# fanzhongyi/ExploreMultiModal

Measured on AMD Instinct MI355X. Metric: image-text pairs/sec fwd+bwd, VLMo-Base, 1/2/4/8 MI355X; % bf16 MFMA roofline, higher is better.
Workload: dtype bf16

## Files before the change

### exploremultimodal_amd/csrc/block.hip

```cpp
#include "common.h"
#include "vlmo_hip.h"
#include <algorithm>
#include <map>
#include <vector>

namespace {
constexpr int GELU_DERIV = 4;


struct Events {
    std::vector<hipEvent_t> pool;
    hipEvent_t get(size_t i) {
        while (pool.size() <= i) {
            hipEvent_t e = nullptr;
            (void)hipEventCreateWithFlags(&e, hipEventDisableTiming);
            pool.push_back(e);
        }
        return pool[i];
    }
};
Events& events() {
    static thread_local std::map<int, Events> per_device;
    int dev = 0;
    (void)hipGetDevice(&dev);
// ... 289 lines not shown
    arm();
    TRY(vlmo_ln_bwd(b->dy1, 0, nullptr, b->x, b->n1w, b->mean1, b->rstd1, b->dx1, b->dx0, b->dn1w, b->dn1b, M, d,
                    ws_slot(2 + b->n_experts), slot, st));
    collect();
    return 0;
}

}

extern "C" int vlmo_stack_fwd(const VlmoStackDesc* s, hipStream_t st) {
    VLMO_CHECK_ARG(s && s->blocks && s->n_blocks >= 1, "vlmo_stack_fwd: empty stack");
    for (int i = 0; i < s->n_blocks; ++i)
        if (int rc = block_fwd(&s->blocks[i], st)) return rc;
    return 0;
}

extern "C" int vlmo_stack_bwd(const VlmoStackDesc* s, hipStream_t st) {
    VLMO_CHECK_ARG(s && s->blocks && s->n_blocks >= 1, "vlmo_stack_bwd: empty stack");
    const int nb = s->n_blocks;
    const int batch = s->wgrad_batch >= 1 ? s->wgrad_batch : 1;
    const int nsets = s->n_tmp_sets >= 1 ? s->n_tmp_sets : 1;
    hipStream_t side = s->side_stream ? s->side_stream : st;
    const bool two = side != st;
    VLMO_CHECK_ARG(!two || nsets > batch || nb <= nsets,
                   "vlmo_stack_bwd: %d temporary sets cannot cover deferred batches of %d blocks", nsets, batch);
    Events& ev = events();
    Deferred D;
    D.store = s->wgrad_store != 0;
    std::vector<int> batch_of(nb, -1);
    int n_batches = 0, waited_upto = -1;
    auto flush = [&]() -> int {
        if (D.blocks.empty()) return 0;
        if (two) {
            hipEvent_t f = ev.get(2 * n_batches);
            (void)hipEventRecord(f, st);
            (void)hipStreamWaitEvent(side, f, 0);
        }
        std::stable_sort(D.tn.begin(), D.tn.end(), [](const VlmoTnProblem& a, const VlmoTnProblem& b) { return a.M > b.M; });
        TRY(vlmo_gemm_tn_multi(VLMO_BF16, D.tn.data(), (int)D.tn.size(), side));
        TRY(vlmo_colwork_multi(VLMO_BF16, D.col.data(), (int)D.col.size(), side));
        if (two) (void)hipEventRecord(ev.get(2 * n_batches + 1), side);
        if (s->grad_ready)
            for (int i : D.blocks)
                if (s->grad_ready[i]) (void)hipEventRecord((hipEvent_t)s->grad_ready[i], side);
        ++n_batches;
        D.tn.clear();
        D.col.clear();
// ... 49 lines not shown
```

### exploremultimodal_amd/csrc/gemm_tn.hip

```cpp
#include "gemm_common.h"
#include <algorithm>
#include <vector>

namespace {

struct GemmTN {
    const void* A;
    const void* B;
    float* C;
    int M, N1, N2, lda, ldb, ldc;
    int kt_per_split, tiles;
    float alpha;
    float* slab;
    int mode;
};
enum { TN_ATOMIC = 0, TN_ACCUM = 1, TN_STORE = 2 };

__device__ __attribute__((aligned(256))) char tn_zero_page[256];

__device__ __forceinline__ int tn_swz(int row) { return ((row & 3) << 2) | ((row >> 2) & 3); }

template <typename T, int BM, int BN, int WM, int WN, bool PP = false>
__device__ __forceinline__ void gemm_tn_body(const GemmTN& p, const int lid) {
    typedef typename Elem<T>::v8 v8;
// ... 217 lines not shown
        for (int j = 0; j < TN; ++j) {
            const int gn = n2_0 + wn * (BN / WN) + j * 32 + l31;
#pragma unroll
            for (int r = 0; r < 16; ++r) {
                const int gm = n1_0 + wm * (BM / WM) + i * 32 + (r & 3) + 8 * (r >> 2) + 4 * h;
                if (gm < p.N1 && gn < p.N2) {
                    float* c = p.C + (size_t)gm * p.ldc + gn;
                    if (p.slab)
                        p.slab[((size_t)split * p.N1 + gm) * p.N2 + gn] = acc[i][j][r];
                    else if (p.mode == TN_STORE)
                        *c = p.alpha * acc[i][j][r];
                    else
                        atomicAdd(c, p.alpha * acc[i][j][r]);
                }
            }
        }
}

template <typename T, int BM, int BN, int WM, int WN, bool PP = false>
__global__ __launch_bounds__(WM * WN * 64, 2) void gemm_tn_kernel(const GemmTN p) {
    gemm_tn_body<T, BM, BN, WM, WN, PP>(p, xcd_remap(blockIdx.x, gridDim.x));
}

constexpr int MAX_TN_PROBS = 16;
constexpr int MAX_TN_ORDER = 1024;
constexpr uint16_t TN_NOP = 0xFFFF;
struct GemmTNMulti {
    int n;
    GemmTN p[MAX_TN_PROBS];
    uint16_t order[MAX_TN_ORDER];
};
template <typename T>
__global__ __launch_bounds__(512, 2) void gemm_tn_multi_kernel(const GemmTNMulti mp) {
    const uint32_t code = mp.order[blockIdx.x];
    if (code == TN_NOP) return;
    int gi = (int)(code >> 12);
    const int lid_in = __builtin_amdgcn_readfirstlane((int)(code & 0xFFFu));
    gi = __builtin_amdgcn_readfirstlane(gi);
    const GemmTN& q = mp.p[gi];
    GemmTN p;
    p.A = uniform_ptr(q.A), p.B = uniform_ptr(q.B), p.C = (float*)uniform_ptr(q.C);
    p.M = __builtin_amdgcn_readfirstlane(q.M), p.N1 = __builtin_amdgcn_readfirstlane(q.N1);
    p.N2 = __builtin_amdgcn_readfirstlane(q.N2), p.lda = __builtin_amdgcn_readfirstlane(q.lda);
    p.ldb = __builtin_amdgcn_readfirstlane(q.ldb), p.ldc = __builtin_amdgcn_readfirstlane(q.ldc);
    p.kt_per_split = __builtin_amdgcn_readfirstlane(q.kt_per_split), p.tiles = __builtin_amdgcn_readfirstlane(q.tiles);
    p.alpha = __builtin_bit_cast(float, __builtin_amdgcn_readfirstlane(__builtin_bit_cast(int, q.alpha)));
    p.slab = nullptr;
    p.mode = __builtin_amdgcn_readfirstlane(q.mode);
    gemm_tn_body<T, 256, 256, 2, 4, true>(p, lid_in);
}

__global__ __launch_bounds__(256) void tn_reduce_kernel(const float* __restrict__ slab, int splits, int N1, int N2,
                                                        float* __restrict__ C, int ldc, float alpha) {
    const int n4 = N2 >> 2;
    const long total = (long)N1 * n4;
    for (long i = (long)blockIdx.x * 256 + threadIdx.x; i < total; i += (long)gridDim.x * 256) {
        const int r = (int)(i / n4), c = (int)(i % n4) * 4;
        f32x4 a = {0.f, 0.f, 0.f, 0.f};
        for (int s2 = 0; s2 < splits; ++s2) a += *(const f32x4*)(slab + ((size_t)s2 * N1 + r) * N2 + c);
        f32x4* o = (f32x4*)(C + (size_t)r * ldc + c);
        *o = *o + alpha * a;
    }
// ... 58 lines not shown
            (void)hipFuncSetAttribute((const void*)gemm_tn_kernel<bf16, 256, 256, 2, 4, true>, hipFuncAttributeMaxDynamicSharedMemorySize, LDS);
            (void)hipFuncSetAttribute((const void*)gemm_tn_kernel<f16, 256, 256, 2, 4, true>, hipFuncAttributeMaxDynamicSharedMemorySize, LDS);
        }
        if (dtype == VLMO_F16)
            hipLaunchKernelGGL((gemm_tn_kernel<f16, 256, 256, 2, 4, true>), grid, dim3(512), LDS, stream, p);
        else
            hipLaunchKernelGGL((gemm_tn_kernel<bf16, 256, 256, 2, 4, true>), grid, dim3(512), LDS, stream, p);
    } else {
        if (dtype == VLMO_F16)
            hipLaunchKernelGGL((gemm_tn_kernel<f16, 128, 128, 2, 2>), grid, dim3(256), 65536, stream, p);
        else
            hipLaunchKernelGGL((gemm_tn_kernel<bf16, 128, 128, 2, 2>), grid, dim3(256), 65536, stream, p);
    }
    VLMO_CHECK_LAUNCH("vlmo_gemm_tn");
    if (use_slab) {
        const long total = (long)N1 * (N2 / 4);
        const int rg = (int)((total + 255) / 256 < 2048 ? (total + 255) / 256 : 2048);
        hipLaunchKernelGGL(tn_reduce_kernel, dim3(rg), dim3(256), 0, stream, ws, pl.splits, N1, N2, C, ldc, alpha);
        VLMO_CHECK_LAUNCH("vlmo_gemm_tn(reduce)");
    }
    return 0;
}

extern "C" int vlmo_gemm_tn_multi(int dtype, const VlmoTnProblem* probs, int n, hipStream_t stream) {
    VLMO_CHECK_ARG(probs && n >= 1, "vlmo_gemm_tn_multi: no problems");
    VLMO_CHECK_ARG(dtype == VLMO_BF16 || dtype == VLMO_F16, "vlmo_gemm_tn_multi: dtype must be bf16 or f16");
    static DeviceOnce attr;
    if (attr.first()) {
        constexpr int LDS = 2 * 4 * 64 * 256;
        (void)hipFuncSetAttribute((const void*)gemm_tn_multi_kernel<bf16>, hipFuncAttributeMaxDynamicSharedMemorySize, LDS);
        (void)hipFuncSetAttribute((const void*)gemm_tn_multi_kernel<f16>, hipFuncAttributeMaxDynamicSharedMemorySize, LDS);
    }
    for (int q0 = 0, nq = 0; q0 < n; q0 += nq) {
        nq = 0;
        for (long tl = 0; q0 + nq < n && nq < MAX_TN_PROBS; ++nq) {
            const VlmoTnProblem& r = probs[q0 + nq];
            const long t = (long)((r.N1 + 255) / 256) * ((r.N2 + 255) / 256);
            if (nq > 0 && tl + t > MAX_TN_ORDER - 64) break;
            tl += t;
        }
        long tiles_all = 0;
        int min_nk = 1 << 30;
        double flops = 0;
        for (int q = 0; q < nq; ++q) {
            const VlmoTnProblem& r = probs[q0 + q];
            VLMO_CHECK_ARG(r.A && r.B && r.C, "vlmo_gemm_tn_multi: null operand in problem %d", q0 + q);
            VLMO_CHECK_ARG(r.M > 0 && r.N1 >= 8 && r.N2 >= 8 && r.N1 % 8 == 0 && r.N2 % 8 == 0 && r.lda % 8 == 0 &&
                               r.ldb % 8 == 0 && r.lda >= r.N1 && r.ldb >= r.N2 && r.ldc >= r.N2,
                           "vlmo_gemm_tn_multi: bad shape in problem %d (M=%d N1=%d N2=%d)", q0 + q, r.M, r.N1, r.N2);
            tiles_all += (long)((r.N1 + 255) / 256) * ((r.N2 + 255) / 256);
            const int nk = (r.M + 63) / 64;
            if (nk < min_nk) min_nk = nk;
            flops += 2.0 * r.M * r.N1 * r.N2;
        }
        int splits = 1;
        if (tiles_all < 192) {
            splits = (int)(256 / tiles_all);
            if (splits > min_nk / 8) splits = min_nk / 8;
            if (splits < 1) splits = 1;
        }
        GemmTNMulti mp{};
        mp.n = nq;
        struct Job {
            uint16_t code;
            int cost;
        };
        std::vector<Job> jobs;
        for (int q = 0; q < nq; ++q) {
            const VlmoTnProblem& r = probs[q0 + q];
            const int tiles = ((r.N1 + 255) / 256) * ((r.N2 + 255) / 256);
            const int nk = (r.M + 63) / 64;
            int sp = splits > nk ? nk : splits;
            const int per = (nk + sp - 1) / sp;
            sp = (nk + per - 1) / per;
            int mode = r.accumulate ? TN_ACCUM : TN_STORE;
            if (sp > 1) {
                mode = TN_ATOMIC;
                if (!r.accumulate) {
                    hipError_t rc = hipMemset2DAsync(r.C, (size_t)r.ldc * 4, 0, (size_t)r.N2 * 4, r.N1, stream);
                    if (rc != hipSuccess) {
                        vlmo_set_error("vlmo_gemm_tn_multi: memset failed: %s", hipGetErrorString(rc));
                        return (int)rc;
                    }
                }
            }
            VLMO_CHECK_ARG(tiles * sp <= 4096, "vlmo_gemm_tn_multi: problem %d has too many tiles", q0 + q);
            mp.p[q] = GemmTN{r.A, r.B, r.C, r.M, r.N1, r.N2, r.lda, r.ldb, r.ldc, per, tiles, r.alpha, nullptr, mode};
            for (int l = 0; l < tiles * sp; ++l) jobs.push_back(Job{(uint16_t)((q << 12) | l), per});
        }
        std::stable_sort(jobs.begin(), jobs.end(), [](const Job& a, const Job& b) { return a.cost > b.cost; });
        std::vector<uint16_t> bins[8];
        for (size_t i = 0; i < jobs.size();) {
            size_t j = i;
            while (j < jobs.size() && jobs[j].cost == jobs[i].cost) ++j;
            const size_t cnt = j - i;
            for (int x = 0; x < 8; ++x)
                for (size_t k = i + cnt * x / 8; k < i + cnt * (x + 1) / 8; ++k) bins[x].push_back(jobs[k].code);
            i = j;
        }
        size_t deepest = 0;
        for (int x = 0; x < 8; ++x) deepest = bins[x].size() > deepest ? bins[x].size() : deepest;
        VLMO_CHECK_ARG(deepest * 8 <= (size_t)MAX_TN_ORDER, "vlmo_gemm_tn_multi: %zu workgroups exceed one launch (pass fewer problems per call)",
                       jobs.size());
        const int t = (int)deepest * 8;
        for (int b = 0; b < t; ++b) {
            const std::vector<uint16_t>& bin = bins[b & 7];
            mp.order[b] = (size_t)(b >> 3) < bin.size() ? bin[b >> 3] : TN_NOP;
        }
        ProfScope prof(73, flops, stream);
        constexpr int LDS = 2 * 4 * 64 * 256;
        if (dtype == VLMO_F16)
            hipLaunchKernelGGL((gemm_tn_multi_kernel<f16>), dim3(t), dim3(512), LDS, stream, mp);
        else
            hipLaunchKernelGGL((gemm_tn_multi_kernel<bf16>), dim3(t), dim3(512), LDS, stream, mp);
        VLMO_CHECK_LAUNCH("vlmo_gemm_tn_multi");
    }
    return 0;
}
```

### exploremultimodal_amd/engine.py

```python
import ctypes
import os as _os
import sys
from collections import namedtuple

import torch

from . import hip

LN_EPS = 1e-12
GRAD_SINK = None
_ov = _os.environ.get('VLMO_OVERLAP_WGRAD')
OVERLAP_WGRAD = None if _ov is None else _ov != '0'
ONE_STREAM_ROWS = 12288


def _use_side_stream(sink, rows):
    if OVERLAP_WGRAD is not None:
        return OVERLAP_WGRAD
    return sink is not None or rows < ONE_STREAM_ROWS


DEFAULT_TILE = -1


# ... 304 lines not shown
    return [(w1, 0), (b1, hid * d), (w2, hid * d + hid), (b2, 2 * hid * d + hid)]


def _fill_grads(D, flats, d, hid, nexp):
    (dg1, dg2, dn1w, dn1b, dn2w, dn2b, dqkv_w, dproj_w, dproj_b, dqkv_b) = _carve(
        flats[0], [(d,)] * 6 + [(3 * d, d), (d, d), (d,), (3 * d,)])
    D.dg1, D.dg2, D.dn1w, D.dn1b, D.dn2w, D.dn2b = (t.data_ptr() for t in (dg1, dg2, dn1w, dn1b, dn2w, dn2b))
    D.dqkv_w, D.dproj_w, D.dproj_b, D.dqkv_b = (t.data_ptr() for t in (dqkv_w, dproj_w, dproj_b, dqkv_b))
    dexp = []
    for i in range(nexp):
        dw1, db1, dw2, db2 = _carve(flats[1 + i], [(hid, d), (hid,), (d, hid), (d,)])
        D.dw1[i], D.db1[i], D.dw2[i], D.db2[i] = dw1.data_ptr(), db1.data_ptr(), dw2.data_ptr(), db2.data_ptr()
        dexp += [dw1, db1, dw2, db2]
    return [dg1, dg2, dn1w, dn1b, dqkv_w, dqkv_b[:d], dqkv_b[2 * d:], dproj_w, dproj_b, dn2w, dn2b] + dexp


def _released(ctx_field):
    if ctx_field is None:
        raise RuntimeError('Trying to backward through an engine pass a second time: its saved activations were released '
                           'by the first backward (retain_graph=True is not supported by engine.StackFn)')


WGRAD_BATCH = int(_os.environ.get('VLMO_WGRAD_BATCH', '2'))


def wgrad_batch_for(d, hid, cus=256, max_batch=4):
    if WGRAD_BATCH > 0:
        return WGRAD_BATCH
    c = lambda n: -(-n // 256)
    tiles = c(d) * c(3 * d) + c(d) * c(d) + 2 * c(d) * c(hid)
    best, best_cost = 1, None
    for b in range(1, max_batch + 1):
        cost = -(-b * tiles // cus) / b
        if best_cost is None or cost < best_cost - 1e-9:
            best, best_cost = b, cost
    return best


TMP_SETS = 4
USE_STACK = True

_PERSIST = {}


def _persist(dev, tag, numel, dtype):
    key = (dev, torch.cuda.current_stream(dev).cuda_stream, tag)
    t = _PERSIST.get(key)
    if t is None or t.numel() < numel or t.dtype != dtype:
        t = _PERSIST[key] = torch.empty(numel, dtype=dtype, device=dev)
    return t


_EVENTS = {}


def _ready_events(dev, n):
    evs = _EVENTS.setdefault(dev, [])
    while len(evs) < n:
        evs.append(hip.event_create())
# ... 102 lines not shown
    if base is None or g.dtype != torch.float32 or base.dim() != 1 or not base.is_contiguous():
        return None
    off = (g.data_ptr() - base.data_ptr()) // 4
    if off < 0 or off + n > base.numel():
        return None
    return base[off:off + n]


def _same_views(layout, flat):
    for p_, off in layout:
        if not p_.requires_grad:
            continue
        pg = p_.grad
        if pg is None or pg.data_ptr() != flat.data_ptr() + 4 * off or not pg.is_contiguous() or pg.dtype != torch.float32:
            return False
        if getattr(p_, '_post_accumulate_grad_hooks', None) or getattr(p_, '_backward_hooks', None):
            return False
    return True


_Scratch = namedtuple('_Scratch', 'nsets batch tb ws ws_n dxs')


def _backward_scratch(dev, nb, M, d, hid, B):
    want = wgrad_batch_for(d, hid)
    nsets = max(1, min(max(TMP_SETS, want + 1), nb))
    batch = max(1, min(want, nsets - 1)) if nb > nsets else max(1, want)
    md = M * d
    tb = _persist(dev, 'tb', nsets * 11 * md, torch.bfloat16)
    slot = hip.lib().vlmo_reduce_ws_bytes(2 * d)
    ws_n = 6 * slot // 4 + (M // 16 + 4) * hid + 4 * B * d
    ws = _persist(dev, 'ws', nsets * ws_n, torch.float32)
    dxs = _persist(dev, 'dx', 3 * md, torch.float32)
    return _Scratch(nsets, batch, tb, ws, ws_n, dxs)


def _sink_buckets(sink, groups, d, hid, dev):
    akey = id(groups[0].params[0])
    aroom = group_numel(groups[0], d, hid) + ARENA_EXPERTS * group_numel(groups[1], d, hid)
    return [sink.acquire(g.params, group_numel(g, d, hid), dev, akey, aroom, layout=group_layout(g, d, hid), lazy_zero=True)
            for g in groups]


FRESH, FROM_TASK, FROM_GRAD = 0, 1, 2


def _local_bucket(g, d, hid, wanted, reg, permitted, into_grad, fresh):
    key = _group_key(g.params)
    if wanted:
        if reg is not None and key in reg:
            return reg[key], FROM_TASK
        if into_grad:
            have = _grad_flat(g.params, group_numel(g, d, hid))
            if have is not None and _same_views(group_layout(g, d, hid), have):
# ... 117 lines not shown
            ctx.metas, ctx.descs, ctx.keep, ctx.spans, ctx.groups = metas, descs, keep, spans, groups
            ctx.save_for_backward(x, *params)
            ctx.sink = GRAD_SINK
            if ctx.sink is None:
                ctx.grad_groups = [(_group_key(g.params), g.params) for blk in groups for g in blk]
            else:
                ctx.sink_groups = [[g.params for g in blk] for blk in groups]
                for blk in ctx.sink_groups:
                    for gp in blk:
                        ctx.sink.expect(gp)
        return out

    @staticmethod
    def backward(ctx, dxo):
        metas, descs, spans, groups = ctx.metas, ctx.descs, ctx.spans, ctx.groups
        _released(descs)
        x, *params = ctx.saved_tensors
        nb = len(metas)
        m0 = metas[0]
        d, hid = m0.d, m0.hidden
        M, dev = x.shape[0], x.device
        dxo = dxo.contiguous()
        sink = ctx.sink
        sc = _backward_scratch(dev, nb, M, d, hid, m0.plan.B)
        dx_in = torch.empty((M, d), dtype=torch.float32, device=dev)
        if sink is None:
            storage = _fresh_storage(sum(group_numel(g, d, hid) for blk in groups for g in blk), dev)
            reg = _task_flats(ctx) if INPLACE_ACCUM else None
            permitted, into_grad, off = _TASK_FLATS['groups'], INPLACE_ACCUM and _INTO_GRAD[0], 0
        grads_all = [None] * len(params)
        store_ok, acquired = True, []
        for k in range(nb):
            i = nb - 1 - k
            D, blk, (o, n_) = descs[i], groups[i], spans[i]
            if sink is not None:
                got = _sink_buckets(sink, blk, d, hid, dev)
            else:
                got, off = _local_buckets(blk, ctx.needs_input_grad[2 + o:2 + o + n_], d, hid, reg, permitted, into_grad,
                                          storage, off)
            store_ok = store_ok and all(fr for _, fr in got)
            acquired += [(f_, fr, g.lo > 0) for g, (f_, fr) in zip(blk, got)]
            grads = _fill_grads(D, [f_ for f_, _ in got], d, hid, len(blk) - 1)
            for g, (_, fr) in zip(blk, got):
                if fr or sink is not None:
                    grads_all[o + g.lo:o + g.hi] = grads[g.lo:g.hi]
            _split_backward_attention(D, metas[i])
            _wire_temporaries(D, k, nb, M * d, sc, dxo, dx_in)
        _zero_buckets(acquired, store_ok, d, hid)
        S = hip.StackDesc()
        S.n_blocks, S.wgrad_batch, S.n_tmp_sets, S.wgrad_store = nb, sc.batch, sc.nsets, int(store_ok)
        S.blocks = ctypes.cast(descs, ctypes.POINTER(hip.BlockDesc))
        side = _side_stream(dev) if _use_side_stream(sink, M) else None
        S.side_stream = side.cuda_stream if side is not None else None
        evs = None
        if sink is not None and side is not None:
            evs = _ready_events(dev, nb)
            arr = (ctypes.c_void_p * nb)(*evs)
            S.grad_ready = ctypes.cast(arr, ctypes.POINTER(ctypes.c_void_p))
        hip.stack_bwd(S)
        ctx.descs = ctx.keep = None
        if sink is not None:
            _hand_to_sink(sink, groups, spans, grads_all, evs)
            return (dx_in, None) + (None,) * len(params)
        return (dx_in, None, *grads_all)


class FinalNormFn(torch.autograd.Function):

    @staticmethod
    def forward(ctx, x, w, b, plan, out_shape, eps=LN_EPS):
        M, d = x.shape
        out = torch.empty(out_shape, dtype=torch.float32, device=x.device)
        mean, rstd = torch.empty(M, device=x.device), torch.empty(M, device=x.device)
        hip.ln_fwd(x, w, b, out, mean, rstd, plan.rowmap, M, d, eps)
        ctx.plan = plan
# ... 91 lines not shown
```

### exploremultimodal_amd/hip.py

```python
import ctypes
import os

import torch

_HERE = os.path.dirname(os.path.abspath(__file__))
LIB_PATH = os.environ.get('VLMO_HIP_LIB') or os.path.join(_HERE, 'lib', 'libvlmo_hip.so')

BF16, F16, F32 = 0, 1, 2
EPI_BIAS, EPI_BIAS_GELU, EPI_RESID, EPI_DGELU, EPI_F32, EPI_DUAL, EPI_ARGMAX, EPI_CE, EPI_CE_BWD = 0, 1, 2, 3, 4, 5, 6, 7, 8

_vp, _i32, _u32, _u64, _f32, _i64 = (ctypes.c_void_p, ctypes.c_int32, ctypes.c_uint32,
                                     ctypes.c_uint64, ctypes.c_float, ctypes.c_int64)


class Epilogue(ctypes.Structure):
    _fields_ = [('out', _vp), ('out2', _vp), ('bias', _vp), ('gamma', _vp),
                ('resid', _vp), ('row_scale', _vp), ('row_index', _vp), ('aux', _vp),
                ('ldo', _i32), ('ld2', _i32), ('relu', _i32),
                ('drop_thresh', _u32), ('inv_keep', _f32), ('beta', _f32),
                ('seed', _u64), ('colpart', _vp)]


_fp = _vp

# ... 59 lines not shown
    'vlmo_resid_bwd': [_vp, _vp, _vp, _vp, _vp, _vp, _vp, _vp, _i32, _i32, _u32, _f32, _u64, _vp, _i64, _vp],
    'vlmo_colsum': [_i32, _vp, _i32, _vp, _i32, _i32, _vp, _i64, _vp],
    'vlmo_cast_weight': [_i32, _vp, _i32, _i32, _vp, _vp, _vp],
    'vlmo_cast_weight_multi': [_i32, _i32, _vp, _vp, _vp, _vp, _vp, _vp],
    'vlmo_patchify': [_vp, _vp, _i32, _i32, _i32, _i32, _i32, _vp],
    'vlmo_embed_img_finish': [_vp, _vp, _vp, _vp, _vp, _vp, _vp, _i32, _i32, _i32, _u32, _f32,
                              _u64, _vp],
    'vlmo_embed_img_bwd': [_vp, _vp, _vp, _vp, _vp, _vp, _vp, _i32, _i32, _i32, _u32, _f32,
                           _u64, _vp],
    'vlmo_embed_txt_fwd': [_vp] * 10 + [_i32, _i32, _i32, _f32, _u32, _f32, _u64, _vp],
    'vlmo_embed_txt_bwd': [_vp] * 11 + [_i32, _i32, _i32, _u32, _f32, _u64, _vp],
    'vlmo_conv2d_nhwc': [_i32, _i32, _vp, _i32, _i32, _i32, _i32, _i32, _vp, _i32, _vp,
                         ctypes.POINTER(Epilogue), _vp],
    'vlmo_dvae_im2col': [_vp, _vp, _i32, _i32, _i32, _i32, _i32, _i32, _vp],
    'vlmo_maxpool2_nhwc': [_vp, _vp, _vp, _i32, _i32, _i32, _i32, _vp],
    'vlmo_argmax_reduce': [_vp, _i32, _vp, _i32, _vp],
    'vlmo_dvae_embed': [_vp, _vp, _vp, _vp, _i32, _i32, _i32, _vp],
    'vlmo_upsample2_nhwc': [_vp, _vp, _i32, _i32, _i32, _i32, _vp],
    'vlmo_dvae_out_head': [_vp, _vp, _vp, _vp, _i32, _i32, _i32, _i32, _i32, _vp],
    'vlmo_ce_reduce': [_vp, _i32, _vp, _i32, _vp, _vp, _vp, _i32, _vp],
    'vlmo_stack_fwd': [ctypes.POINTER(StackDesc), _vp],
    'vlmo_stack_bwd': [ctypes.POINTER(StackDesc), _vp],
    'vlmo_gemm_tn_multi': [_i32, ctypes.POINTER(TnProblem), _i32, _vp],
    'vlmo_colwork_multi': [_i32, ctypes.POINTER(ColJob), _i32, _vp],
    'vlmo_event_create': [ctypes.POINTER(ctypes.c_void_p)],
    'vlmo_event_destroy': [_vp],
    'vlmo_stream_wait_event': [_vp, _vp],
    'vlmo_profile_start': [_i32],
    'vlmo_gemm_nt_grouped': [_i32, _i32, _i32, _i32, _vp, _i32, _vp, _i32, _vp, _i32, _i32, _vp, _vp],
    'vlmo_mt_grad_norm': [ctypes.c_void_p, _f32, _f32, _vp, _vp, _vp],
    'vlmo_mt_adam': [ctypes.c_void_p, ctypes.c_void_p, _vp, _vp],
    'vlmo_mt_ema': [ctypes.c_void_p, _f32, _vp],
    'vlmo_mt_adam_ema': [ctypes.c_void_p, ctypes.c_void_p, _vp, _vp, _f32, _vp],
    'vlmo_side_stream_create': [_i32, ctypes.POINTER(ctypes.c_uint32), _i32, ctypes.POINTER(ctypes.c_void_p)],
    'vlmo_profile_stop': [_i32, ctypes.POINTER(ctypes.c_double), ctypes.POINTER(ctypes.c_double),
                          ctypes.POINTER(ctypes.c_int64)],
    'vlmo_gemm_nt_2src': [_i32, _i32, _i32, _vp, _i32, _i32, _f32, _vp, _i32, _vp, _i32, _i32, _i32, _i32,
                          ctypes.POINTER(Epilogue), _vp],
    'vlmo_comm_available': [],
    'vlmo_comm_unique_id': [_vp],
    'vlmo_comm_init': [ctypes.POINTER(ctypes.c_void_p), _vp, _i32, _i32],
    'vlmo_comm_destroy': [_vp],
    'vlmo_comm_count': [_vp, _vp, _vp],
    'vlmo_comm_all_reduce': [_vp, _vp, _vp, _i64, _i32, _vp],
    'vlmo_comm_reduce_scatter': [_vp, _vp, _vp, _i64, _i32, _vp],
    'vlmo_comm_all_gather': [_vp, _vp, _vp, _i64, _i32, _vp],
    'vlmo_grad_pack': [_vp, _vp, _i64, _f32, _vp],
    'vlmo_grad_unpack': [_vp, _vp, _i64, _vp],
    'vlmo_ln_gelu_fwd': [_vp, _i32, _vp, _vp, _vp, _i32, _vp, _vp, _i32, _i32, _f32, _vp],
    'vlmo_ln_gelu_bwd': [_vp, _i32, _vp, _i32, _vp, _vp, _vp, _vp, _vp, _i32, _vp, _i32, _vp, _vp, _vp, _i32, _i32, _vp,
                         _i64, _vp],
    'vlmo_vqa_bce': [_vp, _i32, _vp, _i32, _i32, _i32, _vp, _vp, _vp, _vp, _f32, _vp, _i32, _vp, _i32, _vp],
    'vlmo_isda_update': [_vp, _i32, _vp, _vp, _vp, _vp, _vp, _i32, _i32, _i32, _i32, _vp, _vp, _vp, _vp, _vp],
    'vlmo_isda_aug_fwd': [_vp, _i32, _vp, _vp, _i32, _i32, _i32, _i32, _f32, _vp, _i32, _vp, _i64, _vp],
    'vlmo_isda_aug_bwd': [_vp, _i32, _vp, _i32, _vp, _vp, _i32, _i32, _i32, _i32, _f32, _vp, _i32, _vp, _i64, _vp],
    'vlmo_sim_topk': [_vp, _i32, _vp, _i32, _i32, _i32, _i32, _i32, _f32, _i32, _vp, ctypes.c_size_t, _vp, _vp, _vp],
    'vlmo_crop_resample': [_vp, _i64, _vp, _vp, _i32, _vp, _vp, _i32, ctypes.POINTER(_f32), ctypes.POINTER(_f32), _f32, _vp,
                           _i64, _vp],
}

_lib = None
ABI_VERSION = 9

def lib():
    global _lib
    if _lib is None:
        if not os.path.exists(LIB_PATH):
            raise RuntimeError(
                f'{LIB_PATH} not found: build the HIP extension first '
                '(python -c "import __graft_entry__ as g; g.build()" or '
                'make -C exploremultimodal_amd/csrc). There is no CPU fallback.')
        L = ctypes.CDLL(LIB_PATH)
        L.vlmo_last_error.restype = ctypes.c_char_p
        L.vlmo_abi_version.restype = ctypes.c_int
        if L.vlmo_abi_version() != ABI_VERSION:
            raise RuntimeError(f'{LIB_PATH} has ABI version {L.vlmo_abi_version()}, this package needs {ABI_VERSION}: '
                               'rebuild it (make -C exploremultimodal_amd/csrc)')
        L.vlmo_reduce_ws_bytes.restype = ctypes.c_int64
        L.vlmo_reduce_ws_bytes.argtypes = [_i32]
        L.vlmo_gemm_tn_ws_bytes.restype = ctypes.c_int64
        L.vlmo_isda_ws_bytes.restype = ctypes.c_int64
        L.vlmo_isda_ws_bytes.argtypes = [_i32, _i32, _i32]
        L.vlmo_gemm_tn_ws_bytes.argtypes = [_i32, _i32, _i32]
        L.vlmo_sim_topk_ws_bytes.restype = ctypes.c_int64
        L.vlmo_sim_topk_ws_bytes.argtypes = [_i32, _i32, _i32, _i32]
# ... 246 lines not shown
def dvae_embed(ids, table, bias, out):
    vocab, n_init = table.shape
    _check(lib().vlmo_dvae_embed(_p(ids), _p(table), _p(bias), _p(out), ids.numel(), vocab, n_init, _stream()),
           'vlmo_dvae_embed')


def upsample2_nhwc(x, out, B, H, W, C):
    _check(lib().vlmo_upsample2_nhwc(_p(x), _p(out), B, H, W, C, _stream()), 'vlmo_upsample2_nhwc')


def dvae_out_head(x, w, bias, out, B, H, W):
    Cout, C = w.shape
    _check(lib().vlmo_dvae_out_head(_p(x), _p(w), _p(bias), _p(out), B, H, W, C, Cout, _stream()), 'vlmo_dvae_out_head')


def gemm_tn_multi(problems, dtype=BF16):
    n = len(problems)
    arr = (TnProblem * n)()
    for i, (A, B, C, M, N1, N2, acc) in enumerate(problems):
        arr[i] = TnProblem(_p(A), _p(B), _p(C), A.stride(0), B.stride(0), C.stride(0), M, N1, N2, 1.0, int(acc))
    _check(lib().vlmo_gemm_tn_multi(dtype, arr, n, _stream()), 'vlmo_gemm_tn_multi')


def colwork_multi(jobs, dtype=BF16):
    n = len(jobs)
    arr = (ColJob * n)()
    for i, (kind, src, rows, ncols, outs, n0) in enumerate(jobs):
        o = (ctypes.c_void_p * 4)(*[_p(t) for t in (list(outs) + [None] * 4)[:4]])
        arr[i] = ColJob(kind, src.stride(0), _p(src), rows, ncols, o, n0, 0)
    _check(lib().vlmo_colwork_multi(dtype, arr, n, _stream()), 'vlmo_colwork_multi')


def event_create():
    out = ctypes.c_void_p()
    _check(lib().vlmo_event_create(ctypes.byref(out)), 'vlmo_event_create')
    return out.value


def stream_wait_event(stream, ev):
    raw = stream.cuda_stream if hasattr(stream, 'cuda_stream') else stream
    _check(lib().vlmo_stream_wait_event(raw, ev), 'vlmo_stream_wait_event')


COMM_ID_BYTES = 128


# ... 253 lines not shown
```

### include/vlmo_hip.h

```cpp
#ifndef VLMO_HIP_H
#define VLMO_HIP_H

#include <stddef.h>
#include <stdint.h>

#ifdef __cplusplus
extern "C" {
#endif

#ifndef __HIP_PLATFORM_AMD__
typedef struct ihipStream_t* hipStream_t;
#endif

enum { VLMO_BF16 = 0, VLMO_F16 = 1, VLMO_F32 = 2 };

enum {
    VLMO_EPI_BIAS = 0,
    VLMO_EPI_BIAS_GELU = 1,
    VLMO_EPI_RESID = 2,
    VLMO_EPI_DGELU = 3,
    VLMO_EPI_F32 = 4,
    VLMO_EPI_DUAL = 5,
    VLMO_EPI_ARGMAX = 6,
    VLMO_EPI_CE = 7,
    VLMO_EPI_CE_BWD = 8
};

typedef struct VlmoEpilogue {
    void* out;
    void* out2;
    const float* bias;
    const float* gamma;
    const float* resid;
    const float* row_scale;
    const int32_t* row_index;
    const void* aux;
    int32_t ldo, ld2;
    int32_t relu;
    uint32_t drop_thresh;
    float inv_keep;
    float beta;
    uint64_t seed;
    float* colpart;
} VlmoEpilogue;

const char* vlmo_last_error(void);
#define VLMO_ABI_VERSION 9
int vlmo_abi_version(void);

int vlmo_gemm_nt(int epi, int dtype, int tile, const void* A, int lda, const void* B, int ldb,
                 int M, int N, int K, const VlmoEpilogue* e, hipStream_t stream);
int vlmo_gemm_nt_2src(int epi, int dtype, int tile, const void* A, int lda, int k1, float seg_scale, const void* A2,
                      int lda2, const void* B, int ldb, int M, int N, int K, const VlmoEpilogue* e,
                      hipStream_t stream);
int vlmo_gemm_nt_grouped(int epi, int dtype, int tile, int ngroups, const void* const* A, int lda,
                         const void* const* B, int ldb, const int32_t* M, int N, int K,
                         const VlmoEpilogue* e, hipStream_t stream);

int64_t vlmo_gemm_tn_ws_bytes(int M, int N1, int N2);
int vlmo_gemm_tn(int dtype, const void* A, int lda, const void* B, int ldb, float* C, int ldc,
                 int M, int N1, int N2, float alpha, int splits, float* ws, int64_t ws_bytes,
                 hipStream_t stream);

typedef struct VlmoTnProblem {
    const void* A;
    const void* B;
    float* C;
    int32_t lda, ldb, ldc;
    int32_t M, N1, N2;
    float alpha;
    int32_t accumulate;
} VlmoTnProblem;
int vlmo_gemm_tn_multi(int dtype, const VlmoTnProblem* probs, int n, hipStream_t stream);

int vlmo_ln_fwd(const float* x, const float* w, const float* b, void* y, int out_f32,
                float* mean, float* rstd, const int32_t* rowmap, int M, int d, float eps,
                hipStream_t stream);
int64_t vlmo_reduce_ws_bytes(int ncols);

int vlmo_ln_bwd(const void* dy, int dy_f32, const int32_t* rowmap, const float* x, const float* w,
                const float* mean, const float* rstd, const float* dres, float* dx, float* dw,
                float* db, int M, int d, float* ws, int64_t ws_bytes, hipStream_t stream);

int vlmo_ln_resid_bwd(const void* dy, const float* x, const float* w, const float* mean, const float* rstd,
                      const float* dres, float* dx, float* dw, float* db, const void* zd, const float* gamma,
                      const float* row_scale, const int32_t* row_index, void* dz, float* dgamma, float* dbias,
                      uint32_t drop_thresh, float inv_keep, uint64_t seed, int M, int d, float* ws,
                      int64_t ws_bytes, hipStream_t stream);

int vlmo_attn_fwd(const void* qkv, const int32_t* seg, int num_seq, const int32_t* keymask,
                  void* ctx, float* lse, int lse_stride, int heads, int d, int max_len,
                  float scale, uint32_t drop_thresh, float inv_keep, uint64_t seed, int mask_seq0,
                  hipStream_t stream);
int vlmo_attn_bwd(const void* qkv, const void* ctx, const void* dctx, const float* lse,
                  int lse_stride, const int32_t* seg, int num_seq, const int32_t* keymask,
                  void* dqkv, float* qv_colsum, int heads, int d, int max_len, float scale,
// ... 204 lines not shown
```

Measured before the change: 4538.

## Cache grouped wgrad GEMM tables on device and size single-stream wgrad batches by makespan

Moves the grouped TN weight-gradient GEMM's problem table and workgroup order from a kernel-argument struct into a device buffer. Plans are cached per device, stream and problem set, so repeated calls skip re-planning and re-uploading, and one launch now handles any number of problems instead of chunks of 16. When no side stream is used, the backward pass picks the deferred wgrad batch size from a predicted makespan over CU slots, bounded by a temporary-memory cap. This adds pinned/device allocations, a hash-keyed LRU cache, and more scratch memory when all blocks are batched at once.

```diff
diff --git a/exploremultimodal_amd/csrc/block.hip b/exploremultimodal_amd/csrc/block.hip
--- a/exploremultimodal_amd/csrc/block.hip
+++ b/exploremultimodal_amd/csrc/block.hip
@@ -335,7 +335,7 @@
     const int nsets = s->n_tmp_sets >= 1 ? s->n_tmp_sets : 1;
     hipStream_t side = s->side_stream ? s->side_stream : st;
     const bool two = side != st;
-    VLMO_CHECK_ARG(!two || nsets > batch || nb <= nsets,
+    VLMO_CHECK_ARG(nsets > batch || nb <= nsets,
                    "vlmo_stack_bwd: %d temporary sets cannot cover deferred batches of %d blocks", nsets, batch);
     Events& ev = events();
     Deferred D;
diff --git a/exploremultimodal_amd/csrc/gemm_tn.hip b/exploremultimodal_amd/csrc/gemm_tn.hip
--- a/exploremultimodal_amd/csrc/gemm_tn.hip
+++ b/exploremultimodal_amd/csrc/gemm_tn.hip
@@ -1,5 +1,7 @@
 #include "gemm_common.h"
 #include <algorithm>
+#include <cstring>
+#include <mutex>
 #include <vector>
 
 namespace {
@@ -263,22 +265,15 @@
     gemm_tn_body<T, BM, BN, WM, WN, PP>(p, xcd_remap(blockIdx.x, gridDim.x));
 }
 
-constexpr int MAX_TN_PROBS = 16;
-constexpr int MAX_TN_ORDER = 1024;
-constexpr uint16_t TN_NOP = 0xFFFF;
-struct GemmTNMulti {
-    int n;
-    GemmTN p[MAX_TN_PROBS];
-    uint16_t order[MAX_TN_ORDER];
-};
+constexpr int TN_LID_BITS = 16;
 template <typename T>
-__global__ __launch_bounds__(512, 2) void gemm_tn_multi_kernel(const GemmTNMulti mp) {
-    const uint32_t code = mp.order[blockIdx.x];
-    if (code == TN_NOP) return;
-    int gi = (int)(code >> 12);
-    const int lid_in = __builtin_amdgcn_readfirstlane((int)(code & 0xFFFu));
-    gi = __builtin_amdgcn_readfirstlane(gi);
-    const GemmTN& q = mp.p[gi];
+__global__ __launch_bounds__(512, 2) void gemm_tn_multi_kernel(const GemmTN* __restrict__ probs,
+                                                               const uint32_t* __restrict__ order, const int n_wg) {
+    if ((int)blockIdx.x >= n_wg) return;
+    const uint32_t code = order[blockIdx.x];
+    const int gi = __builtin_amdgcn_readfirstlane((int)(code >> TN_LID_BITS));
+    const int lid_in = __builtin_amdgcn_readfirstlane((int)(code & ((1u << TN_LID_BITS) - 1)));
+    const GemmTN& q = probs[gi];
     GemmTN p;
     p.A = uniform_ptr(q.A), p.B = uniform_ptr(q.B), p.C = (float*)uniform_ptr(q.C);
     p.M = __builtin_amdgcn_readfirstlane(q.M), p.N1 = __builtin_amdgcn_readfirstlane(q.N1);
@@ -383,98 +378,219 @@
     return 0;
 }
 
+namespace {
+
+constexpr int TN_CACHE_PER_STREAM = 32;
+
+struct TnClear {
+    float* C;
+    int ldc, N1, N2;
+};
+struct TnTable {
+    int device = -1;
+    hipStream_t stream = nullptr;
+    uint64_t hash = 0, used = 0;
+    std::vector<VlmoTnProblem> key;
+    char* dev = nullptr;
+    char* host = nullptr;
+    size_t cap = 0, order_off = 0;
+    hipEvent_t uploaded = nullptr;
+    int n_wg = 0;
+    double flops = 0;
+    std::vector<TnClear> clears;
+};
+struct TnCache {
+    std::mutex mu;
+    std::vector<TnTable*> tables;
+    uint64_t clock = 0;
+    int64_t uploads = 0, hits = 0;
+};
+TnCache& tn_cache() {
+    static TnCache* c = new TnCache;
+    return *c;
+}
+static_assert(sizeof(VlmoTnProblem) == 56, "VlmoTnProblem has padding: compare the cache key field by field");
+
+uint64_t tn_hash(const VlmoTnProblem* probs, int n) {
+    const uint64_t* w = (const uint64_t*)probs;
+    uint64_t h = 0xcbf29ce484222325ull ^ (uint64_t)n;
+    for (size_t i = 0; i < (size_t)n * (sizeof(VlmoTnProblem) / 8); ++i) h = (h ^ w[i]) * 0x100000001b3ull;
+    return h;
+}
+
+int tn_plan_multi(const VlmoTnProblem* probs, int n, std::vector<GemmTN>& recs, std::vector<uint32_t>& order,
+                  std::vector<TnClear>& clears, double* flops_out) {
+    long tiles_all = 0;
+    int min_nk = 1 << 30;
+    double flops = 0;
+    VLMO_CHECK_ARG(n < (1 << (32 - TN_LID_BITS)), "vlmo_gemm_tn_multi: %d problems exceed one call", n);
+    for (int q = 0; q < n; ++q) {
+        const VlmoTnProblem& r = probs[q];
+        VLMO_CHECK_ARG(r.A && r.B && r.C, "vlmo_gemm_tn_multi: null operand in problem %d", q);
+        VLMO_CHECK_ARG(r.M > 0 && r.N1 >= 8 && r.N2 >= 8 && r.N1 % 8 == 0 && r.N2 % 8 == 0 && r.lda % 8 == 0 &&
+                           r.ldb % 8 == 0 && r.lda >= r.N1 && r.ldb >= r.N2 && r.ldc >= r.N2,
+                       "vlmo_gemm_tn_multi: bad shape in problem %d (M=%d N1=%d N2=%d)", q, r.M, r.N1, r.N2);
+        tiles_all += (long)((r.N1 + 255) / 256) * ((r.N2 + 255) / 256);
+        const int nk = (r.M + 63) / 64;
+        if (nk < min_nk) min_nk = nk;
+        flops += 2.0 * r.M * r.N1 * r.N2;
+    }
+    int splits = 1;
+    if (tiles_all < 192) {
+        splits = (int)(256 / tiles_all);
+        if (splits > min_nk / 8) splits = min_nk / 8;
+        if (splits < 1) splits = 1;
+    }
+    struct Job {
+        uint32_t code;
+        int cost;
+    };
+    std::vector<Job> jobs;
+    jobs.reserve((size_t)tiles_all * splits);
+    recs.clear();
+    clears.clear();
+    for (int q = 0; q < n; ++q) {
+        const VlmoTnProblem& r = probs[q];
+        const long tiles = (long)((r.N1 + 255) / 256) * ((r.N2 + 255) / 256);
+        const int nk = (r.M + 63) / 64;
+        int sp = splits > nk ? nk : splits;
+        const int per = (nk + sp - 1) / sp;
+        sp = (nk + per - 1) / per;
+        int mode = r.accumulate ? TN_ACCUM : TN_STORE;
+        if (sp > 1) {
+            mode = TN_ATOMIC;
+            if (!r.accumulate) clears.push_back(TnClear{r.C, r.ldc, r.N1, r.N2});
+        }
+        VLMO_CHECK_ARG(tiles * sp <= (1L << TN_LID_BITS), "vlmo_gemm_tn_multi: problem %d has too many tiles", q);
+        recs.push_back(GemmTN{r.A, r.B, r.C, r.M, r.N1, r.N2, r.lda, r.ldb, r.ldc, per, (int)tiles, r.alpha, nullptr, mode});
+        for (int l = 0; l < (int)tiles * sp; ++l) jobs.push_back(Job{((uint32_t)q << TN_LID_BITS) | (uint32_t)l, per});
+    }
+    std::stable_sort(jobs.begin(), jobs.end(), [](const Job& a, const Job& b) { return a.cost > b.cost; });
+    std::vector<uint32_t> bins[8];
+    int first = 0;
+    for (size_t i = 0; i < jobs.size();) {
+        size_t j = i;
+        while (j < jobs.size() && jobs[j].cost == jobs[i].cost) ++j;
+        const size_t cnt = j - i, k = cnt / 8, r = cnt % 8;
+        size_t at = i;
+        for (int x = 0; x < 8; ++x) {
+            std::vector<uint32_t>& bin = bins[(first + x) & 7];
+            for (size_t e = 0, len = k + ((size_t)x < r ? 1 : 0); e < len; ++e) bin.push_back(jobs[at++].code);
+        }
+        first = (first + (int)r) & 7;
+        i = j;
+    }
+    order.resize(jobs.size());
+    for (size_t b = 0; b < order.size(); ++b) order[b] = bins[b & 7][b >> 3];
+    *flops_out = flops;
+    return 0;
+}
+
+}
+
+extern "C" int vlmo_tn_table_stats(int64_t* uploads, int64_t* hits, int64_t* entries) {
+    TnCache& c = tn_cache();
+    std::lock_guard<std::mutex> lock(c.mu);
+    if (uploads) *uploads = c.uploads;
+    if (hits) *hits = c.hits;
+    if (entries) *entries = (int64_t)c.tables.size();
+    return 0;
+}
+
 extern "C" int vlmo_gemm_tn_multi(int dtype, const VlmoTnProblem* probs, int n, hipStream_t stream) {
     VLMO_CHECK_ARG(probs && n >= 1, "vlmo_gemm_tn_multi: no problems");
     VLMO_CHECK_ARG(dtype == VLMO_BF16 || dtype == VLMO_F16, "vlmo_gemm_tn_multi: dtype must be bf16 or f16");
+    constexpr int LDS = 2 * 4 * 64 * 256;
     static DeviceOnce attr;
     if (attr.first()) {
-        constexpr int LDS = 2 * 4 * 64 * 256;
         (void)hipFuncSetAttribute((const void*)gemm_tn_multi_kernel<bf16>, hipFuncAttributeMaxDynamicSharedMemorySize, LDS);
         (void)hipFuncSetAttribute((const void*)gemm_tn_multi_kernel<f16>, hipFuncAttributeMaxDynamicSharedMemorySize, LDS);
     }
-    for (int q0 = 0, nq = 0; q0 < n; q0 += nq) {
-        nq = 0;
-        for (long tl = 0; q0 + nq < n && nq < MAX_TN_PROBS; ++nq) {
-            const VlmoTnProblem& r = probs[q0 + nq];
-            const long t = (long)((r.N1 + 255) / 256) * ((r.N2 + 255) / 256);
-            if (nq > 0 && tl + t > MAX_TN_ORDER - 64) break;
-            tl += t;
-        }
-        long tiles_all = 0;
-        int min_nk = 1 << 30;
+    int device = 0;
+    (void)hipGetDevice(&device);
+    const uint64_t hash = tn_hash(probs, n);
+    TnCache& c = tn_cache();
+    std::lock_guard<std::mutex> lock(c.mu);
+    TnTable* t = nullptr;
+    int mine = 0;
+    for (TnTable* e : c.tables) {
+        if (e->device != device || e->stream != stream) continue;
+        ++mine;
+        if (e->hash == hash && (int)e->key.size() == n && memcmp(e->key.data(), probs, (size_t)n * sizeof(VlmoTnProblem)) == 0) {
+            t = e;
+            break;
+        }
+    }
+    if (t) {
+        ++c.hits;
+    } else {
+        std::vector<GemmTN> recs;
+        std::vector<uint32_t> order;
+        std::vector<TnClear> clears;
         double flops = 0;
-        for (int q = 0; q < nq; ++q) {
-            const VlmoTnProblem& r = probs[q0 + q];
-            VLMO_CHECK_ARG(r.A && r.B && r.C, "vlmo_gemm_tn_multi: null operand in problem %d", q0 + q);
-            VLMO_CHECK_ARG(r.M > 0 && r.N1 >= 8 && r.N2 >= 8 && r.N1 % 8 == 0 && r.N2 % 8 == 0 && r.lda % 8 == 0 &&
-                               r.ldb % 8 == 0 && r.lda >= r.N1 && r.ldb >= r.N2 && r.ldc >= r.N2,
-                           "vlmo_gemm_tn_multi: bad shape in problem %d (M=%d N1=%d N2=%d)", q0 + q, r.M, r.N1, r.N2);
-            tiles_all += (long)((r.N1 + 255) / 256) * ((r.N2 + 255) / 256);
-            const int nk = (r.M + 63) / 64;
-            if (nk < min_nk) min_nk = nk;
-            flops += 2.0 * r.M * r.N1 * r.N2;
-        }
-        int splits = 1;
-        if (tiles_all < 192) {
-            splits = (int)(256 / tiles_all);
-            if (splits > min_nk / 8) splits = min_nk / 8;
-            if (splits < 1) splits = 1;
-        }
-        GemmTNMulti mp{};
-        mp.n = nq;
-        struct Job {
-            uint16_t code;
-            int cost;
-        };
-        std::vector<Job> jobs;
-        for (int q = 0; q < nq; ++q) {
-            const VlmoTnProblem& r = probs[q0 + q];
-            const int tiles = ((r.N1 + 255) / 256) * ((r.N2 + 255) / 256);
-            const int nk = (r.M + 63) / 64;
-            int sp = splits > nk ? nk : splits;
-            const int per = (nk + sp - 1) / sp;
-            sp = (nk + per - 1) / per;
-            int mode = r.accumulate ? TN_ACCUM : TN_STORE;
-            if (sp > 1) {
-                mode = TN_ATOMIC;
-                if (!r.accumulate) {
-                    hipError_t rc = hipMemset2DAsync(r.C, (size_t)r.ldc * 4, 0, (size_t)r.N2 * 4, r.N1, stream);
-                    if (rc != hipSuccess) {
-                        vlmo_set_error("vlmo_gemm_tn_multi: memset failed: %s", hipGetErrorString(rc));
-                        return (int)rc;
-                    }
-                }
-            }
-            VLMO_CHECK_ARG(tiles * sp <= 4096, "vlmo_gemm_tn_multi: problem %d has too many tiles", q0 + q);
-            mp.p[q] = GemmTN{r.A, r.B, r.C, r.M, r.N1, r.N2, r.lda, r.ldb, r.ldc, per, tiles, r.alpha, nullptr, mode};
-            for (int l = 0; l < tiles * sp; ++l) jobs.push_back(Job{(uint16_t)((q << 12) | l), per});
-        }
-        std::stable_sort(jobs.begin(), jobs.end(), [](const Job& a, const Job& b) { return a.cost > b.cost; });
-        std::vector<uint16_t> bins[8];
-        for (size_t i = 0; i < jobs.size();) {
-            size_t j = i;
-            while (j < jobs.size() && jobs[j].cost == jobs[i].cost) ++j;
-            const size_t cnt = j - i;
-            for (int x = 0; x < 8; ++x)
-                for (size_t k = i + cnt * x / 8; k < i + cnt * (x + 1) / 8; ++k) bins[x].push_back(jobs[k].code);
-            i = j;
-        }
-        size_t deepest = 0;
-        for (int x = 0; x < 8; ++x) deepest = bins[x].size() > deepest ? bins[x].size() : deepest;
-        VLMO_CHECK_ARG(deepest * 8 <= (size_t)MAX_TN_ORDER, "vlmo_gemm_tn_multi: %zu workgroups exceed one launch (pass fewer problems per call)",
-                       jobs.size());
-        const int t = (int)deepest * 8;
-        for (int b = 0; b < t; ++b) {
-            const std::vector<uint16_t>& bin = bins[b & 7];
-            mp.order[b] = (size_t)(b >> 3) < bin.size() ? bin[b >> 3] : TN_NOP;
-        }
-        ProfScope prof(73, flops, stream);
-        constexpr int LDS = 2 * 4 * 64 * 256;
-        if (dtype == VLMO_F16)
-            hipLaunchKernelGGL((gemm_tn_multi_kernel<f16>), dim3(t), dim3(512), LDS, stream, mp);
-        else
-            hipLaunchKernelGGL((gemm_tn_multi_kernel<bf16>), dim3(t), dim3(512), LDS, stream, mp);
-        VLMO_CHECK_LAUNCH("vlmo_gemm_tn_multi");
-    }
+        if (int rc = tn_plan_multi(probs, n, recs, order, clears, &flops)) return rc;
+        const size_t order_off = recs.size() * sizeof(GemmTN), need = order_off + order.size() * 4;
+        if (mine >= TN_CACHE_PER_STREAM) {
+            for (TnTable* e : c.tables)
+                if (e->device == device && e->stream == stream && (!t || e->used < t->used) &&
+                    hipEventQuery(e->uploaded) == hipSuccess)
+                    t = e;
+            (void)hipGetLastError();
+        }
+        if (!t) {
+            t = new TnTable;
+            t->device = device, t->stream = stream;
+            hipError_t rc = hipEventCreateWithFlags(&t->uploaded, hipEventDisableTiming);
+            if (rc != hipSuccess) {
+                delete t;
+                vlmo_set_error("vlmo_gemm_tn_multi: event: %s", hipGetErrorString(rc));
+                return (int)rc;
+            }
+            c.tables.push_back(t);
+        }
+        t->hash = 0, t->key.clear();
+        if (t->cap < need) {
+            if (t->dev) (void)hipFree(t->dev);
+            if (t->host) (void)hipHostFree(t->host);
+            t->dev = t->host = nullptr, t->cap = 0;
+            const size_t cap = (need + 4095) & ~(size_t)4095;
+            hipError_t rc = hipMalloc((void**)&t->dev, cap);
+            if (rc == hipSuccess) rc = hipHostMalloc((void**)&t->host, cap, hipHostMallocDefault);
+            if (rc != hipSuccess) {
+                vlmo_set_error("vlmo_gemm_tn_multi: table of %zu bytes: %s", cap, hipGetErrorString(rc));
+                return (int)rc;
+            }
+            t->cap = cap;
+        }
+        memcpy(t->host, recs.data(), order_off);
+        memcpy(t->host + order_off, order.data(), order.size() * 4);
+        hipError_t rc = hipMemcpyAsync(t->dev, t->host, need, hipMemcpyHostToDevice, stream);
+        if (rc == hipSuccess) rc = hipEventRecord(t->uploaded, stream);
+        if (rc != hipSuccess) {
+            vlmo_set_error("vlmo_gemm_tn_multi: table upload failed: %s", hipGetErrorString(rc));
+            return (int)rc;
+        }
+        t->order_off = order_off, t->n_wg = (int)order.size(), t->flops = flops;
+        t->clears.swap(clears);
+        t->key.assign(probs, probs + n);
+        t->hash = hash;
+        ++c.uploads;
+    }
+    t->used = ++c.clock;
+    for (const TnClear& z : t->clears) {
+        hipError_t rc = hipMemset2DAsync(z.C, (size_t)z.ldc * 4, 0, (size_t)z.N2 * 4, z.N1, stream);
+        if (rc != hipSuccess) {
+            vlmo_set_error("vlmo_gemm_tn_multi: memset failed: %s", hipGetErrorString(rc));
+            return (int)rc;
+        }
+    }
+    const GemmTN* d_probs = (const GemmTN*)t->dev;
+    const uint32_t* d_order = (const uint32_t*)(t->dev + t->order_off);
+    ProfScope prof(73, t->flops, stream);
+    if (dtype == VLMO_F16)
+        hipLaunchKernelGGL((gemm_tn_multi_kernel<f16>), dim3(t->n_wg), dim3(512), LDS, stream, d_probs, d_order, t->n_wg);
+    else
+        hipLaunchKernelGGL((gemm_tn_multi_kernel<bf16>), dim3(t->n_wg), dim3(512), LDS, stream, d_probs, d_order, t->n_wg);
+    VLMO_CHECK_LAUNCH("vlmo_gemm_tn_multi");
     return 0;
 }
diff --git a/exploremultimodal_amd/engine.py b/exploremultimodal_amd/engine.py
--- a/exploremultimodal_amd/engine.py
+++ b/exploremultimodal_amd/engine.py
@@ -1,4 +1,6 @@
 import ctypes
+import functools
+import heapq
 import os as _os
 import sys
 from collections import namedtuple
@@ -350,6 +352,8 @@
 
 
 WGRAD_BATCH = int(_os.environ.get('VLMO_WGRAD_BATCH', '2'))
+WGRAD_BATCH_FORCED = 'VLMO_WGRAD_BATCH' in _os.environ
+WGRAD_TMP_BYTES = 8 << 30
 
 
 def wgrad_batch_for(d, hid, cus=256, max_batch=4):
@@ -363,6 +367,37 @@
         if best_cost is None or cost < best_cost - 1e-9:
             best, best_cost = b, cost
     return best
+
+
+def block_tile_classes(M, d, hid, expert_rows):
+    c = lambda n: -(-n // 256)
+    kt = lambda r: -(-r // 64)
+    return ((c(3 * d) * c(d) + c(d) * c(d), kt(M)),) + tuple((2 * c(d) * c(hid), kt(r)) for r in expert_rows)
+
+
+@functools.lru_cache(maxsize=None)
+def predicted_makespan(blocks, batch, cus=256):
+    total = 0
+    for k0 in range(0, len(blocks), batch):
+        tiles = sorted((kt for blk in blocks[k0:k0 + batch] for n, kt in blk for _ in range(n)), reverse=True)
+        if len(tiles) <= cus:
+            total += tiles[0]
+            continue
+        free_at = [0] * cus
+        for t in tiles:
+            heapq.heapreplace(free_at, free_at[0] + t)
+        total += max(free_at)
+    return total
+
+
+def one_stream_batch(blocks, set_bytes, cap=None):
+    nb = len(blocks)
+    cap = WGRAD_TMP_BYTES if cap is None else cap
+    if nb * set_bytes <= cap:
+        return nb, nb
+    max_batch = max(1, min(cap // set_bytes - 1, nb - 1))
+    batch = min(range(1, max_batch + 1), key=lambda b: (predicted_makespan(blocks, b), -b))
+    return batch, min(batch + 1, nb)
 
 
 TMP_SETS = 4
@@ -511,14 +546,20 @@
 _Scratch = namedtuple('_Scratch', 'nsets batch tb ws ws_n dxs')
 
 
-def _backward_scratch(dev, nb, M, d, hid, B):
-    want = wgrad_batch_for(d, hid)
-    nsets = max(1, min(max(TMP_SETS, want + 1), nb))
-    batch = max(1, min(want, nsets - 1)) if nb > nsets else max(1, want)
+def _backward_scratch(dev, metas, M, one_stream):
+    nb, m0 = len(metas), metas[0]
+    d, hid, B = m0.d, m0.hidden, m0.plan.B
     md = M * d
-    tb = _persist(dev, 'tb', nsets * 11 * md, torch.bfloat16)
     slot = hip.lib().vlmo_reduce_ws_bytes(2 * d)
     ws_n = 6 * slot // 4 + (M // 16 + 4) * hid + 4 * B * d
+    if one_stream and not (WGRAD_BATCH_FORCED and WGRAD_BATCH > 0):
+        blocks = tuple(block_tile_classes(M, d, hid, tuple(n for _, n in mt.expert_ranges)) for mt in reversed(metas))
+        batch, nsets = one_stream_batch(blocks, 11 * md * 2 + ws_n * 4)
+    else:
+        want = wgrad_batch_for(d, hid)
+        nsets = max(1, min(max(TMP_SETS, want + 1), nb))
+        batch = max(1, min(want, nsets - 1)) if nb > nsets else max(1, want)
+    tb = _persist(dev, 'tb', nsets * 11 * md, torch.bfloat16)
     ws = _persist(dev, 'ws', nsets * ws_n, torch.float32)
     dxs = _persist(dev, 'dx', 3 * md, torch.float32)
     return _Scratch(nsets, batch, tb, ws, ws_n, dxs)
@@ -682,7 +723,8 @@
         M, dev = x.shape[0], x.device
         dxo = dxo.contiguous()
         sink = ctx.sink
-        sc = _backward_scratch(dev, nb, M, d, hid, m0.plan.B)
+        side = _side_stream(dev) if _use_side_stream(sink, M) else None
+        sc = _backward_scratch(dev, metas, M, side is None)
         dx_in = torch.empty((M, d), dtype=torch.float32, device=dev)
         if sink is None:
             storage = _fresh_storage(sum(group_numel(g, d, hid) for blk in groups for g in blk), dev)
@@ -710,7 +752,6 @@
         S = hip.StackDesc()
         S.n_blocks, S.wgrad_batch, S.n_tmp_sets, S.wgrad_store = nb, sc.batch, sc.nsets, int(store_ok)
         S.blocks = ctypes.cast(descs, ctypes.POINTER(hip.BlockDesc))
-        side = _side_stream(dev) if _use_side_stream(sink, M) else None
         S.side_stream = side.cuda_stream if side is not None else None
         evs = None
         if sink is not None and side is not None:
diff --git a/exploremultimodal_amd/hip.py b/exploremultimodal_amd/hip.py
--- a/exploremultimodal_amd/hip.py
+++ b/exploremultimodal_amd/hip.py
@@ -105,6 +105,7 @@
     'vlmo_stack_fwd': [ctypes.POINTER(StackDesc), _vp],
     'vlmo_stack_bwd': [ctypes.POINTER(StackDesc), _vp],
     'vlmo_gemm_tn_multi': [_i32, ctypes.POINTER(TnProblem), _i32, _vp],
+    'vlmo_tn_table_stats': [ctypes.POINTER(_i64)] * 3,
     'vlmo_colwork_multi': [_i32, ctypes.POINTER(ColJob), _i32, _vp],
     'vlmo_event_create': [ctypes.POINTER(ctypes.c_void_p)],
     'vlmo_event_destroy': [_vp],
@@ -143,7 +144,7 @@
 }
 
 _lib = None
-ABI_VERSION = 9
+ABI_VERSION = 10
 
 def lib():
     global _lib
@@ -436,6 +437,12 @@
     _check(lib().vlmo_gemm_tn_multi(dtype, arr, n, _stream()), 'vlmo_gemm_tn_multi')
 
 
+def tn_table_stats():
+    u, h, e = _i64(), _i64(), _i64()
+    _check(lib().vlmo_tn_table_stats(ctypes.byref(u), ctypes.byref(h), ctypes.byref(e)), 'vlmo_tn_table_stats')
+    return u.value, h.value, e.value
+
+
 def colwork_multi(jobs, dtype=BF16):
     n = len(jobs)
     arr = (ColJob * n)()
diff --git a/include/vlmo_hip.h b/include/vlmo_hip.h
--- a/include/vlmo_hip.h
+++ b/include/vlmo_hip.h
@@ -45,7 +45,7 @@
 } VlmoEpilogue;
 
 const char* vlmo_last_error(void);
-#define VLMO_ABI_VERSION 9
+#define VLMO_ABI_VERSION 10
 int vlmo_abi_version(void);
 
 int vlmo_gemm_nt(int epi, int dtype, int tile, const void* A, int lda, const void* B, int ldb,
@@ -72,6 +72,7 @@
     int32_t accumulate;
 } VlmoTnProblem;
 int vlmo_gemm_tn_multi(int dtype, const VlmoTnProblem* probs, int n, hipStream_t stream);
+int vlmo_tn_table_stats(int64_t* uploads, int64_t* hits, int64_t* entries);
 
 int vlmo_ln_fwd(const float* x, const float* w, const float* b, void* y, int out_f32,
                 float* mean, float* rstd, const int32_t* rowmap, int M, int d, float eps,
```

Result: no change. 4543, median of 3 (+0.1%).
